# zhenfeizhang/falcon-r1cs

Hardware: AMD Instinct MI355X
Metric: falcon1024_verify_with_ntt_r1cs_witnesses_per_sec (higher is better)
Workload: dtype u32; 1 GPU; falcon-1024 full verify-with-ntt witness (NTT ladder + mod_q + pointwise + l2-norm), batch=65536 signatures per GPU per step (BASELINE configs[2] on every GPU); logn=10, batch_per_gpu=65536, chunk=32768, encoding=bls12-381-fr montgomery (arkworks witness_assignment bytes), seed=0x46414c434f4e31, signatures_failing_range_checks=0, ranks_seen=1, hbm_plan_bytes=166888865792, hbm_plan_limit_bytes=259200000000

## Files before the change

### falcon-r1cs_amd/csrc/frw_layout.h

```cpp
#pragma once
#include <hip/hip_runtime.h>
#include <stddef.h>
#include <stdint.h>

namespace frw {

struct Carve {
    char *base;
    size_t off = 0;
    explicit Carve(void *b) : base((char *)b) {}
    template <class T = void>
    T *take(size_t bytes, size_t align = 256)
    {
        T *p = (T *)(base + off);
        off += (bytes + align - 1) & ~(align - 1);
        return p;
    }
    uint32_t *words(size_t count) { return take<uint32_t>(count * 4, 4); }
    void *at() const { return base + off; }
    void align_to(size_t a) { off = (off + a - 1) & ~(a - 1); }
    static size_t up(size_t bytes, size_t a) { return (bytes + a - 1) & ~(a - 1); }
};

constexpr int MSM_C = 16;
constexpr int MSM_W = 16;
constexpr int MSM_BUCKETS = 1 << (MSM_C - 1);
constexpr int MSM_FOLD1_THREADS = 4096;
constexpr int G1_BK_WORDS = 60, G2_BK_WORDS = 116;
constexpr int MSM_SLICES = 32, MSM_SLICES_LONE = 224;
constexpr int WIDE_C = 20, WIDE_W = 13, WIDE_H = 1 << (WIDE_C - MSM_C), WIDE_ROWS = WIDE_W * WIDE_H;
constexpr uint32_t WIDE_MAX_ITEMS = 65536;
constexpr int WIDE_SLICES = 128;
constexpr int WIDE_BINS = 512, WIDE_BIN_BUCKETS = MSM_BUCKETS * WIDE_H / WIDE_BINS, WIDE_ALL_BINS = WIDE_W * WIDE_BINS, WIDE_TILE = 4096;
constexpr int WIDE_PARTS = 32;
constexpr int MSM_MAX_ITEMS = 131072;
constexpr int MSM_MAX_ITEMS_LARGE = 32768 + (32768 * 24 * 2 / 3) / 32 * 33 + 64;
static_assert(MSM_MAX_ITEMS_LARGE % 64 == 0 && MSM_MAX_ITEMS >= 32768 + (32768 * 4 * 2 / 3) / 32 * 33 + 64, "whole wavefronts; the finest split fits");
__host__ __device__ constexpr uint32_t msm_max_items(uint32_t n, bool bare = false)
{
    return !bare && n > (1u << 18) ? (uint32_t)MSM_MAX_ITEMS_LARGE : (uint32_t)MSM_MAX_ITEMS;
}
constexpr int NMSM_C = 8, NMSM_W = 32, NMSM_BUCKETS = 128;
__host__ __device__ constexpr uint32_t nmsm_slices(uint32_t n) { return n > (1u << 18) ? 128u : 16u; }
constexpr int NMSM_TARGET_ITEMS_MIN = 2048, NMSM_TARGET_ITEMS_MAX = 65536;
__host__ __device__ constexpr uint32_t nmsm_target_items(uint32_t n)
{
    const uint32_t t = (n / 128 + 2047) / 2048 * 2048;
    return t < (uint32_t)NMSM_TARGET_ITEMS_MIN ? (uint32_t)NMSM_TARGET_ITEMS_MIN : t > (uint32_t)NMSM_TARGET_ITEMS_MAX ? (uint32_t)NMSM_TARGET_ITEMS_MAX : t;
}
__host__ __device__ constexpr uint32_t nmsm_max_items(uint32_t n) { return nmsm_target_items(n) + 256; }
constexpr int NMSM_ONES_MAX = 4096, NMSM_ONES_MAX_LARGE = 65536;
__host__ __device__ constexpr uint32_t nmsm_ones_max(uint32_t n) { return n > (1u << 18) ? (uint32_t)NMSM_ONES_MAX_LARGE : (uint32_t)NMSM_ONES_MAX; }

static_assert((size_t)MSM_SLICES * 4 <= (size_t)G1_BK_WORDS * 4, "the slice histograms borrow the buckets' memory");
static_assert((size_t)MSM_SLICES_LONE * MSM_BUCKETS <= (size_t)MSM_MAX_ITEMS * G1_BK_WORDS, "... or, for a lone signature, the work items'");
struct MsmBufs {
    uint32_t *counts, *offsets, *order, *item_first, *item_count, *ones_count, *items, *buckets, *partial, *partial_items, *entries, *ones_list, *end;
    int16_t *digits;
    uint32_t *window_sums;
    uint32_t max_items;
    size_t ent_stride, ones_stride, bytes;
};
inline void msm_layout_head(Carve &c, MsmBufs &b, size_t rows, size_t bw)
{
    b.counts = c.words(rows * MSM_BUCKETS); b.offsets = c.words(rows * MSM_BUCKETS);
    b.order = c.words(rows * MSM_BUCKETS); b.item_first = c.words(rows * MSM_BUCKETS);
    b.item_count = c.words(rows * 4); b.ones_count = c.words(rows * 4);
    b.items = c.words(rows * (size_t)b.max_items * 2);
    b.buckets = c.words(rows * (size_t)MSM_BUCKETS * bw);
    b.partial = c.words(rows * (size_t)MSM_FOLD1_THREADS * bw);
}
inline MsmBufs msm_layout(void *ws, size_t rows, uint32_t n, bool bare, size_t bw)
{
    MsmBufs b{};
    Carve c(ws);
    b.max_items = msm_max_items(n, bare);
    b.ent_stride = bare ? (size_t)n : (size_t)MSM_W * n;
    b.ones_stride = bare ? 0 : (size_t)n;
    msm_layout_head(c, b, rows, bw);
    b.partial_items = c.words(rows * (size_t)b.max_items * bw);
    b.entries = c.words(rows * b.ent_stride);
    b.ones_list = c.words(rows * b.ones_stride);
    if (bare) b.digits = (int16_t *)c.words(((size_t)MSM_W * n * 2 + 3) / 4);
    b.end = (uint32_t *)c.at();
    if (bare) { c.align_to(16); b.window_sums = c.words((size_t)MSM_W * bw); }
    b.bytes = Carve::up(c.off, 16);
    return b;
}
struct MsmWideBufs {
    MsmBufs rows;
    uint32_t *partial_plain, *slice_hist, *bin_count, *row_count, *s1, *s0, *window_sums, *entries, *end;
    unsigned long long *row_start, *bin_start;
    uint2 *coarse;
    int32_t *digits;
    size_t bytes;
};
inline MsmWideBufs msm_layout_wide(void *ws, uint32_t n, size_t bw)
{
    constexpr size_t R = WIDE_ROWS;
    MsmWideBufs w{};
    MsmBufs &b = w.rows;
    Carve c(ws);
    b.max_items = WIDE_MAX_ITEMS;
    msm_layout_head(c, b, R, bw);
    w.partial_plain = c.words(R * (size_t)MSM_FOLD1_THREADS * bw);
    b.partial_items = c.words(R * (size_t)b.max_items * bw);
    w.s1 = c.words(R * bw); w.s0 = c.words(R * bw);
    w.window_sums = c.words((size_t)WIDE_W * bw);
    w.row_start = c.take<unsigned long long>(R * 8, 8);
    w.bin_start = c.take<unsigned long long>((size_t)WIDE_ALL_BINS * 8, 8);
    w.row_count = c.words(R); w.bin_count = c.words(WIDE_ALL_BINS);
    w.slice_hist = c.words((size_t)WIDE_W * WIDE_SLICES * WIDE_BINS);
    w.coarse = (uint2 *)c.words((size_t)WIDE_W * n * 2);
    w.entries = c.words((size_t)WIDE_W * n);
    w.digits = (int32_t *)w.entries;
    w.end = (uint32_t *)c.at();
    b.entries = w.entries; b.ones_list = w.end; b.end = w.end;
    w.bytes = Carve::up(c.off, 16);
    return w;
}
inline size_t msm_workspace_per_signature(uint32_t n, bool bare, bool wide, size_t bw)
{
    return wide ? msm_layout_wide(nullptr, n, bw).bytes : msm_layout(nullptr, bare ? MSM_W : 1, n, bare, bw).bytes;
}

struct NmsmBufs {
    uint32_t *slice_hist, *counts, *offsets, *item_first, *items, *item_count, *ones_count, *ones_list, *entries;
    uint32_t *partial_items, *partial_ones, *folded_ones, *bucket_sums;
    uint32_t target, max_items, ones_stride;
    uint32_t n = 0;
    unsigned long long *entry_base = nullptr;
    uint32_t *window_sums = nullptr;
    uint32_t *end = nullptr;
    size_t used = 0, bytes = 0;
};
inline NmsmBufs nmsm_layout(void *ws, size_t cnt, uint32_t n, size_t bw)
{
    NmsmBufs b;
    Carve c(ws);
    b.target = nmsm_target_items(n); b.max_items = nmsm_max_items(n); b.ones_stride = nmsm_ones_max(n) / 64;
    b.slice_hist = c.words(cnt * (size_t)nmsm_slices(n) * NMSM_BUCKETS);
    b.counts = c.words(cnt * NMSM_BUCKETS);
    b.offsets = c.words(cnt * NMSM_BUCKETS);
    b.item_first = c.words(cnt * NMSM_BUCKETS);
    b.items = c.words(cnt * (size_t)b.max_items);
    b.item_count = c.words(cnt * 4);
    b.ones_count = c.words(cnt * 4);
    b.ones_list = c.words(cnt * (size_t)n);
    b.entries = c.words(cnt * (size_t)NMSM_W * n);
    c.align_to(16);
    b.partial_items = c.words(cnt * (size_t)b.max_items * bw);
    b.partial_ones = c.words(cnt * (size_t)b.ones_stride * bw);
    b.folded_ones = c.words(b.ones_stride > 64 ? cnt * (size_t)64 * bw : 0);
    b.bucket_sums = c.words(cnt * (size_t)NMSM_BUCKETS * bw);
    b.end = (uint32_t *)c.at();
    b.used = c.off;
    b.bytes = Carve::up(c.off + 16, 16);
    return b;
}
inline NmsmBufs nmsm_layout_bare(void *ws, size_t tables, uint32_t n, size_t bw, const NmsmBufs *sorted = nullptr)
{
    constexpr size_t WIN = NMSM_W;
    NmsmBufs b;
    Carve c(ws);
    if (sorted) {
        b = *sorted;
    } else {
        b.target = nmsm_target_items(n); b.max_items = nmsm_max_items(n); b.ones_stride = nmsm_ones_max(n) / 64; b.n = n;
        b.entry_base = c.take<unsigned long long>(WIN * 8, 8);
        b.slice_hist = c.words(WIN * (size_t)nmsm_slices(n) * NMSM_BUCKETS);
        b.counts = c.words(WIN * NMSM_BUCKETS);
        b.offsets = c.words(WIN * NMSM_BUCKETS);
        b.item_first = c.words(WIN * NMSM_BUCKETS);
        b.items = c.words(WIN * (size_t)b.max_items);
        b.item_count = c.words(WIN * 4);
        b.ones_count = c.words(4);
    }
    b.partial_items = c.words(tables * WIN * (size_t)b.max_items * bw);
    b.partial_ones = c.words(tables * (size_t)b.ones_stride * bw);
    b.folded_ones = c.words(tables * (size_t)64 * bw);
    b.bucket_sums = c.words(tables * WIN * (size_t)NMSM_BUCKETS * bw);
    b.window_sums = c.words(tables * WIN * bw);
    if (!sorted) {
        b.ones_list = c.words(n);
        b.entries = c.words(WIN * (size_t)n);
    }
    b.end = (uint32_t *)c.at();
    b.used = c.off;
    b.bytes = Carve::up(c.off + 16, 16);
    return b;
}
inline size_t nmsm_workspace_per_signature(uint32_t n, bool bare, size_t bw) { return bare ? nmsm_layout_bare(nullptr, 1, n, bw).bytes : nmsm_layout(nullptr, 1, n, bw).bytes; }

struct Groth16Points { uint32_t *A, *B1, *L, *H, *SA, *RB1; uint64_t *B2, *rs, *split; };
constexpr size_t GROTH16_POINTS_BYTES = 6 * (size_t)G1_BK_WORDS * 4 + 192 + 64 + 64;
inline Groth16Points groth16_points_layout(Carve &c, size_t cnt)
{
    Groth16Points p;
    p.A = c.words(cnt * G1_BK_WORDS); p.B1 = c.words(cnt * G1_BK_WORDS); p.L = c.words(cnt * G1_BK_WORDS);
    p.H = c.words(cnt * G1_BK_WORDS); p.SA = c.words(cnt * G1_BK_WORDS); p.RB1 = c.words(cnt * G1_BK_WORDS);
    p.B2 = c.take<uint64_t>(cnt * 192, 8); p.rs = c.take<uint64_t>(cnt * 64, 8); p.split = c.take<uint64_t>(cnt * 64, 8);
    return p;
}
struct Groth16Bufs { void *qap_ws; uint64_t *h, *zext; char *msm_ws[5]; Groth16Points pts; size_t qap, msm[5], bytes; };
inline Groth16Bufs groth16_layout(void *ws, size_t cnt, size_t qap, size_t domain, size_t nv, const size_t *msm)
{
    Groth16Bufs g{};
    Carve c(ws);
    g.qap = qap;
    g.qap_ws = c.take(cnt * qap, 1);
    g.h = c.take<uint64_t>(cnt * domain * 32, 1);
    g.zext = c.take<uint64_t>(cnt * (nv + 3) * 32, 1);
    for (int i = 0; i < 5; i++) { g.msm[i] = Carve::up(msm[i], 256); g.msm_ws[i] = c.take<char>(cnt * g.msm[i], 1); }
    g.pts = groth16_points_layout(c, cnt);
    g.bytes = Carve::up(c.off, 256);
    return g;
}
struct Groth16Sides { NmsmBufs g1, gb, g2; };
inline Groth16Sides groth16_sides_layout(Carve &c, uint32_t nz, uint32_t b_rows)
{
    Groth16Sides s;
    s.g1 = nmsm_layout_bare(c.at(), 2, nz, G1_BK_WORDS);              c.take(s.g1.used);
    s.gb = nmsm_layout_bare(c.at(), 1, b_rows, G1_BK_WORDS);          c.take(s.gb.used);
    s.g2 = nmsm_layout_bare(c.at(), 1, b_rows, G2_BK_WORDS, &s.gb);   c.take(s.g2.used);
    return s;
}
struct Groth16BareBufs { void *first_ws; uint64_t *h, *zext; Groth16Sides sides; Groth16Points pts; size_t qap, msm_h, bytes; };
inline Groth16BareBufs groth16_layout_bare(void *ws, size_t qap, size_t msm_h, size_t domain, size_t nv, uint32_t nz, uint32_t b_rows)
{
    Groth16BareBufs g{};
    Carve c(ws);
    g.qap = Carve::up(qap, 256); g.msm_h = Carve::up(msm_h, 256);
    g.first_ws = c.take(g.qap > g.msm_h ? g.qap : g.msm_h, 1);
    g.h = c.take<uint64_t>(domain * 32, 1);
    g.zext = c.take<uint64_t>((nv + 3) * 32, 1);
    g.sides = groth16_sides_layout(c, nz, b_rows);
    g.pts = groth16_points_layout(c, 1);
    g.bytes = Carve::up(c.off, 256);
    return g;
}

struct VerifyBufs { uint64_t *decoded, *prepared; int32_t *decode_status, *status; void *msm_ws, *pairing_ws; size_t msm_bytes, bytes; };
inline VerifyBufs verify_layout(void *ws, size_t k, size_t msm_per, bool bare, size_t proof_bytes = 0, size_t pass_bytes = 0, bool wire = false)
{
    VerifyBufs v{};
    Carve c(ws);
    if (wire) { v.decoded = c.take<uint64_t>(384 * k, 8); v.decode_status = c.take<int32_t>(4 * k, 16); }
    v.msm_bytes = msm_per * (bare ? 1 : k);
    v.msm_ws = c.take(v.msm_bytes, 1);
    v.prepared = c.take<uint64_t>(96 * k, 8);
    v.status = c.take<int32_t>(4 * k, 16);
    v.pairing_ws = c.take(k * proof_bytes + pass_bytes, 1);
    v.bytes = c.off;
    return v;
}
struct RerandBufs { uint64_t *scalars; uint32_t *g1_points, *g2_points; uint64_t *decoded; int32_t *decode_status, *encode_status; size_t bytes; };
constexpr size_t RERAND_SCALAR_BYTES = 128;
inline RerandBufs rerand_layout(void *ws, size_t k, bool wire)
{
    RerandBufs b{};
    Carve c(ws);
    b.scalars = c.take<uint64_t>(k * RERAND_SCALAR_BYTES, 16);
    b.g1_points = c.take<uint32_t>(k * 2 * (size_t)G1_BK_WORDS * 4, 16);
    b.g2_points = c.take<uint32_t>(k * (size_t)G2_BK_WORDS * 4, 16);
    if (wire) {
        b.decoded = c.take<uint64_t>(k * 384, 16);
        b.decode_status = c.take<int32_t>(k * 4, 16);
        b.encode_status = c.take<int32_t>(k * 4, 16);
    }
    b.bytes = c.off;
    return b;
}
struct StatementBufs { uint16_t *pk, *hm; int32_t *decode_status; size_t bytes; };
inline StatementBufs statement_layout(void *ws, int logn, size_t batch)
{
    StatementBufs b{};
    Carve c(ws);
    b.pk = c.take<uint16_t>((batch << logn) * 2, 16);
    b.hm = c.take<uint16_t>((batch << logn) * 2, 16);
    b.decode_status = c.take<int32_t>(batch * 4, 16);
    b.bytes = c.off;
    return b;
}
struct FalconVerifyBufs { uint16_t *sig, *pk, *hm; uint8_t *nonce; int32_t *sig_status, *pk_status; size_t bytes; };
inline FalconVerifyBufs falcon_verify_layout(void *ws, int logn, size_t batch)
{
    FalconVerifyBufs b{};
    Carve c(ws);
    b.sig = c.take<uint16_t>((batch << logn) * 2, 16);
    b.pk = c.take<uint16_t>((batch << logn) * 2, 16);
    b.hm = c.take<uint16_t>((batch << logn) * 2, 16);
    b.nonce = c.take<uint8_t>(batch * 40, 16);
    b.sig_status = c.take<int32_t>(batch * 4, 16);
    b.pk_status = c.take<int32_t>(batch * 4, 16);
    b.bytes = c.off;
    return b;
}
constexpr size_t POK_SCAN_BLOCK = 256;
constexpr size_t POK_WIRE_STAGE = 384;
struct PokProveBufs {
    FalconVerifyBufs screen;
    uint32_t *index, *block_sums, *count;
    uint64_t *rs;
    uint64_t *witness, *instance;
    uint16_t *sig, *pk, *hm;
    uint64_t *proofs;
    uint8_t *wire;
    int32_t *witness_status, *wire_status;
    uint32_t *unsatisfied;
    void *groth16_ws;
    size_t fixed_bytes, per_signature_bytes, groth16_bytes, bytes;
};
inline PokProveBufs pok_prove_layout(void *ws, int logn, size_t batch, size_t k, size_t num_witness, size_t groth16_bytes)
{
    PokProveBufs b{};
    Carve c(ws);
    const size_t n = (size_t)1 << logn;
    b.screen = falcon_verify_layout(c.at(), logn, batch);
    c.take(b.screen.bytes, 16);
    b.index = c.take<uint32_t>(batch * 4, 16);
    b.block_sums = c.take<uint32_t>((batch + POK_SCAN_BLOCK - 1) / POK_SCAN_BLOCK * 4, 16);
    b.count = c.take<uint32_t>(16, 16);
    b.rs = c.take<uint64_t>(batch * 64, 16);
    b.fixed_bytes = c.off;
    c.align_to(256);
    const size_t per0 = c.off;
    b.witness = c.take<uint64_t>(k * num_witness * 32, 256);
    b.instance = c.take<uint64_t>(k * (2 * n + 1) * 32, 16);
    b.sig = c.take<uint16_t>(k * n * 2, 16);
    b.pk = c.take<uint16_t>(k * n * 2, 16);
    b.hm = c.take<uint16_t>(k * n * 2, 16);
    b.proofs = c.take<uint64_t>(k * 384, 16);
    b.wire = c.take<uint8_t>(k * POK_WIRE_STAGE, 16);
    b.witness_status = c.take<int32_t>(k * 4, 16);
    b.wire_status = c.take<int32_t>(k * 4, 16);
    b.unsatisfied = c.take<uint32_t>(k * 4, 16);
    b.per_signature_bytes = c.off - per0;
    c.align_to(256);
    b.groth16_ws = c.take(groth16_bytes, 256);
    b.groth16_bytes = groth16_bytes;
    b.bytes = c.off;
    return b;
}
__host__ __device__ constexpr size_t aggregate_pk_len(int g) { return g ? 1793 : 897; }
__host__ __device__ constexpr size_t aggregate_sig_len(int g) { return g ? 1280 : 666; }
struct AggRoute { size_t pk_off, sig_off, nonce_off; };
__host__ __device__ inline AggRoute aggregate_route(int g, size_t k, size_t s)
{
    const size_t other = s - k;
    AggRoute r;
    r.pk_off = k * aggregate_pk_len(g) + other * aggregate_pk_len(g ^ 1);
    r.sig_off = k * aggregate_sig_len(g) + other * aggregate_sig_len(g ^ 1);
    r.nonce_off = s * 40;
    return r;
}
__host__ __device__ inline size_t aggregate_pk_bytes(size_t count9, size_t count10) { return aggregate_route(0, count9, count9 + count10).pk_off; }
__host__ __device__ inline size_t aggregate_sig_bytes(size_t count9, size_t count10) { return aggregate_route(0, count9, count9 + count10).sig_off; }

struct AggregateScreenBufs {
    uint16_t *sig[2], *pk[2], *hm[2];
    int32_t *sig_status[2], *pk_status[2], *status[2];
    uint64_t *norm[2];
    uint8_t *nonce;
    uint32_t *refused;
    size_t bytes;
};
inline AggregateScreenBufs aggregate_screen_layout(void *ws, size_t count9, size_t count10)
{
    AggregateScreenBufs b{};
    Carve c(ws);
    const size_t count[2] = {count9, count10};
    for (int g = 0; g < 2; g++) {
        const size_t row = count[g] * ((size_t)512 << g) * 2;
        b.sig[g] = c.take<uint16_t>(row, 16);
        b.pk[g] = c.take<uint16_t>(row, 16);
        b.hm[g] = c.take<uint16_t>(row, 16);
        b.sig_status[g] = c.take<int32_t>(count[g] * 4, 16);
        b.pk_status[g] = c.take<int32_t>(count[g] * 4, 16);
        b.status[g] = c.take<int32_t>(count[g] * 4, 16);
        b.norm[g] = c.take<uint64_t>(count[g] * 8, 16);
    }
    b.nonce = c.take<uint8_t>((count9 + count10) * 40, 16);
    b.refused = c.take<uint32_t>(16, 16);
    b.bytes = c.off;
    return b;
}
struct AggregateProveBufs {
    AggregateScreenBufs screen;
    uint64_t *set_witness[2], *set_instance[2];
    int32_t *witness_status[2];
    uint64_t *witness, *instance, *proof;
    uint8_t *wire;
    int32_t *wire_status, *statement_status;
    uint32_t *unsatisfied;
    void *groth16_ws;
    size_t num_witness, num_instance;
    size_t groth16_bytes, bytes;
};
inline AggregateProveBufs aggregate_prove_layout(void *ws, size_t count9, size_t count10, size_t groth16_bytes)
{
    AggregateProveBufs b{};
    Carve c(ws);
    const size_t count[2] = {count9, count10};
    b.screen = aggregate_screen_layout(c.at(), count9, count10);
    c.take(b.screen.bytes, 256);
    b.num_instance = 1;
    for (int g = 0; g < 2; g++) {
        const size_t n = (size_t)512 << g, W = 153 * n + (g ? 52 : 50), I = 2 * n + 1;
        c.align_to(256);
        b.set_witness[g] = c.take<uint64_t>(count[g] * W * 32, 256);
        b.set_instance[g] = c.take<uint64_t>(count[g] * I * 32, 16);
        b.witness_status[g] = c.take<int32_t>(count[g] * 4, 16);
        b.num_witness += count[g] * W;
        b.num_instance += count[g] * (I - 1);
    }
    c.align_to(256);
    b.witness = c.take<uint64_t>(b.num_witness * 32, 256);
    b.instance = c.take<uint64_t>(b.num_instance * 32, 16);
    b.proof = c.take<uint64_t>(384, 16);
    b.wire = c.take<uint8_t>(POK_WIRE_STAGE, 16);
    b.wire_status = c.take<int32_t>(4, 16);
    b.unsatisfied = c.take<uint32_t>(4, 16);
    b.statement_status = c.take<int32_t>((count9 + count10) * 4, 16);
    c.align_to(256);
    b.groth16_ws = c.take(groth16_bytes, 256);
    b.groth16_bytes = groth16_bytes;
    b.bytes = c.off;
    return b;
}
template <class SizeFn> size_t proofs_in_flight(size_t batch, size_t bytes, SizeFn size)
{
    if (batch == 0 || size(1) > bytes) return 0;
    size_t lo = 1, hi = batch;
    while (lo < hi) {
        const size_t mid = lo + (hi - lo + 1) / 2;
        if (size(mid) <= bytes) lo = mid;
        else hi = mid - 1;
    }
    return lo;
}

}
```

### falcon-r1cs_amd/csrc/frw_prepare.hip

```cpp
#include <hip/hip_runtime.h>
#include <stdint.h>
#include <algorithm>
#include "frw_device.h"
#include "frw_keccak.h"
#include "frw_layout.h"

namespace frw {

constexpr int SHAKE256_RATE = 136;
constexpr int NONCE_LEN = 40;

__device__ __forceinline__ void hash_to_point_one(int logn, const uint8_t *__restrict__ nonce, const uint8_t *__restrict__ msg, uint64_t o0,
                                         uint64_t o1, uint16_t *__restrict__ out)
{
    const int n = 1 << logn;
    const size_t total = NONCE_LEN + (size_t)(o1 >= o0 ? o1 - o0 : 0);
    uint64_t st[25];
#pragma unroll
    for (int i = 0; i < 25; i++) st[i] = 0;
    for (size_t pos = 0;; pos += SHAKE256_RATE) {
#pragma unroll
        for (int l = 0; l < SHAKE256_RATE / 8; l++) {
            uint64_t w = 0;
#pragma unroll
            for (int b = 0; b < 8; b++) {
                const size_t p = pos + (size_t)(l * 8 + b);
                uint32_t byte = 0;
                if (p < NONCE_LEN) byte = nonce[p];
                else if (p < total) byte = msg[p - NONCE_LEN];
                else if (p == total) byte = 0x1F;
                w |= (uint64_t)byte << (8 * b);
            }
            st[l] ^= w;
        }
        const bool last = total < pos + SHAKE256_RATE;
        if (last) st[16] ^= 0x8000000000000000ull;
        keccak_f1600(st);
        if (last) break;
    }
    int cnt = 0;
    while (cnt < n) {
#pragma unroll
        for (int w = 0; w < SHAKE256_RATE / 2; w++) {
            const uint64_t lane = st[w / 4];
            const int sh = (w % 4) * 16;
            const uint32_t v = (uint32_t)((lane >> sh) & 0xff) << 8 | (uint32_t)((lane >> (sh + 8)) & 0xff);
            if (v < 5 * Q && cnt < n) out[cnt++] = (uint16_t)(v % Q);
        }
        if (cnt < n) keccak_f1600(st);
    }
}

__global__ __launch_bounds__(BLOCK) void hash_to_point_kernel(int logn, size_t batch, const uint8_t *__restrict__ nonces,
                                                              const uint8_t *__restrict__ msgs,
                                                              const uint64_t *__restrict__ msg_off, uint16_t *__restrict__ hm)
{
    const size_t s = (size_t)blockIdx.x * blockDim.x + threadIdx.x;
    if (s >= batch) return;
    const uint64_t o0 = msg_off[s], o1 = msg_off[s + 1];
    hash_to_point_one(logn, nonces + s * NONCE_LEN, msgs + o0, o0, o1, hm + (s << logn));
}

__device__ __forceinline__ uint32_t public_key_coeff(const uint8_t *__restrict__ p, int k)
{
    const int bit = 14 * k, off = bit & 7;
    const uint8_t *q = p + 1 + (bit >> 3);
    uint32_t acc = (uint32_t)q[0] << 16 | (uint32_t)q[1] << 8;
    if (off + 14 > 16) acc |= q[2];
    return (acc >> (24 - 14 - off)) & 0x3fffu;
}

__global__ __launch_bounds__(BLOCK) void decode_public_keys_kernel(int logn, size_t batch, const uint8_t *__restrict__ pk_bytes,
                                                                   uint16_t *__restrict__ pk, int32_t *__restrict__ status)
{
    const int n = 1 << logn;
    const size_t pk_len = 1 + (size_t)14 * n / 8;
    const size_t idx = (size_t)blockIdx.x * blockDim.x + threadIdx.x;
    if (idx >= batch * (size_t)n) return;
    const size_t s = idx >> logn;
    const int k = (int)(idx & (size_t)(n - 1));
    const uint8_t *p = pk_bytes + s * pk_len;
    const uint32_t c = public_key_coeff(p, k);
    pk[idx] = (uint16_t)c;
    if (c >= Q || (k == 0 && p[0] != (uint8_t)logn)) atomicMax(&status[s], ST_DECODE);
}

__device__ __forceinline__ bool decode_signature_one(int logn, const uint8_t *__restrict__ p, size_t sig_len, uint16_t *__restrict__ out,
                                            uint8_t *__restrict__ nonce_out)
{
    const int n = 1 << logn;
    bool ok = sig_len > 1 + NONCE_LEN && p[0] == (uint8_t)(0x30 + logn);
    if (ok && nonce_out)
        for (int i = 0; i < NONCE_LEN; i++) nonce_out[i] = p[1 + i];
    const uint8_t *body = p + 1 + NONCE_LEN;
    const size_t body_len = ok ? sig_len - 1 - NONCE_LEN : 0;
    size_t v = 0;
    uint32_t acc = 0;
    int acc_len = 0;
    for (int u = 0; ok && u < n; u++) {
        if (v >= body_len) { ok = false; break; }
        acc = (acc << 8) | body[v++];
        const uint32_t b = acc >> acc_len;
        const uint32_t sign = b & 128u;
        uint32_t m = b & 127u;
        for (;;) {
            if (acc_len == 0) {
                if (v >= body_len) { ok = false; break; }
                acc = (acc << 8) | body[v++];
                acc_len = 8;
            }
            acc_len--;
            if ((acc >> acc_len) & 1u) break;
            m += 128;
            if (m > 2047) { ok = false; break; }
        }
        if (sign && m == 0) ok = false;
        if (ok) out[u] = (uint16_t)(sign ? Q - m : m);
    }
    if (ok && (acc & ((1u << acc_len) - 1u))) ok = false;
    for (; ok && v < body_len; v++)
        if (body[v]) ok = false;
    return ok;
}

__global__ __launch_bounds__(BLOCK) void decode_signatures_kernel(int logn, size_t batch, const uint8_t *__restrict__ sig_bytes,
                                                                  size_t sig_len, uint16_t *__restrict__ sig,
                                                                  uint8_t *__restrict__ nonce_out, int32_t *__restrict__ status)
{
    const size_t s = (size_t)blockIdx.x * blockDim.x + threadIdx.x;
    if (s >= batch) return;
    const bool ok = decode_signature_one(logn, sig_bytes + s * sig_len, sig_len, sig + (s << logn),
                                         nonce_out ? nonce_out + s * NONCE_LEN : nullptr);
    status[s] = ok ? ST_OK : ST_DECODE;
}

__global__ __launch_bounds__(BLOCK) void agg_hash_to_point_kernel(int logn, size_t count, const uint32_t *__restrict__ stmt,
                                                                  const uint8_t *__restrict__ nonces, const uint8_t *__restrict__ msgs,
                                                                  const uint64_t *__restrict__ msg_off, uint16_t *__restrict__ hm)
{
    const size_t k = (size_t)blockIdx.x * blockDim.x + threadIdx.x;
    if (k >= count) return;
    const size_t s = stmt[k];
    const uint64_t o0 = msg_off[s], o1 = msg_off[s + 1];
    hash_to_point_one(logn, nonces + aggregate_route(logn - 9, k, s).nonce_off, msgs + o0, o0, o1, hm + (k << logn));
}

__global__ __launch_bounds__(BLOCK) void agg_decode_public_keys_kernel(int logn, size_t count, const uint32_t *__restrict__ stmt,
                                                                       const uint8_t *__restrict__ pk_bytes, uint16_t *__restrict__ pk,
                                                                       int32_t *__restrict__ status)
{
    const int n = 1 << logn;
    const size_t idx = (size_t)blockIdx.x * blockDim.x + threadIdx.x;
    if (idx >= count * (size_t)n) return;
    const size_t k = idx >> logn;
    const int j = (int)(idx & (size_t)(n - 1));
    const uint8_t *p = pk_bytes + aggregate_route(logn - 9, k, stmt[k]).pk_off;
    const uint32_t c = public_key_coeff(p, j);
    pk[idx] = (uint16_t)c;
    if (c >= Q || (j == 0 && p[0] != (uint8_t)logn)) atomicMax(&status[k], ST_DECODE);
}

__global__ __launch_bounds__(BLOCK) void agg_decode_signatures_kernel(int logn, size_t count, const uint32_t *__restrict__ stmt,
                                                                      const uint8_t *__restrict__ sig_bytes, uint16_t *__restrict__ sig,
                                                                      uint8_t *__restrict__ nonces, int32_t *__restrict__ status)
{
    const size_t k = (size_t)blockIdx.x * blockDim.x + threadIdx.x;
    if (k >= count) return;
    const AggRoute r = aggregate_route(logn - 9, k, stmt[k]);
    const uint8_t *p = sig_bytes + r.sig_off;
    for (int i = 0; i < NONCE_LEN; i++) nonces[r.nonce_off + i] = p[1 + i];
    status[k] = decode_signature_one(logn, p, aggregate_sig_len(logn - 9), sig + (k << logn), nullptr) ? ST_OK : ST_DECODE;
}

struct AggVerdicts { const uint32_t *stmt[2]; const int32_t *status[2]; const uint64_t *norm[2]; uint32_t count[2]; };
__global__ __launch_bounds__(BLOCK) void agg_scatter_verdicts_kernel(AggVerdicts v, int32_t *__restrict__ status, uint64_t *__restrict__ norm)
{
    size_t k = (size_t)blockIdx.x * blockDim.x + threadIdx.x;
    int g = 0;
    if (k >= v.count[0]) { k -= v.count[0]; g = 1; }
    if (k >= v.count[g]) return;
    const size_t s = v.stmt[g][k];
    status[s] = v.status[g][k];
    if (norm) norm[s] = v.norm[g][k];
}

__global__ __launch_bounds__(BLOCK) void agg_count_refused_kernel(size_t count, const int32_t *__restrict__ status, uint32_t *__restrict__ refused)
{
    __shared__ uint32_t wave_count[WAVES];
    uint32_t mine = 0;
    for (size_t s = threadIdx.x; s < count; s += BLOCK) mine += status[s] != ST_OK;
#pragma unroll
    for (int off = WAVE / 2; off > 0; off >>= 1) mine += __shfl_xor(mine, off, WAVE);
    if ((threadIdx.x & (WAVE - 1)) == 0) wave_count[threadIdx.x / WAVE] = mine;
    __syncthreads();
    if (threadIdx.x == 0) {
        uint32_t total = 0;
#pragma unroll
        for (int w = 0; w < WAVES; w++) total += wave_count[w];
        refused[0] = total;
    }
}


__device__ inline uint32_t pok_block_rank(bool flag, uint32_t &total)
{
    __shared__ uint32_t wave_count[WAVES];
    const uint64_t mask = __ballot(flag);
    const int lane = threadIdx.x & (WAVE - 1), wave = threadIdx.x / WAVE;
    if (lane == 0) wave_count[wave] = (uint32_t)__popcll(mask);
    __syncthreads();
    uint32_t before = 0;
    total = 0;
#pragma unroll
    for (int w = 0; w < WAVES; w++) {
        if (w < wave) before += wave_count[w];
        total += wave_count[w];
    }
    return before + (uint32_t)__popcll(mask & (((uint64_t)1 << lane) - 1));
}

__global__ __launch_bounds__(BLOCK) void pok_scan_count_kernel(size_t batch, const int32_t *__restrict__ status,
                                                               uint32_t *__restrict__ block_sums)
{
    const size_t s = (size_t)blockIdx.x * BLOCK + threadIdx.x;
    uint32_t total;
    (void)pok_block_rank(s < batch && status[s] == ST_OK, total);
    if (threadIdx.x == 0) block_sums[blockIdx.x] = total;
}

__global__ __launch_bounds__(BLOCK) void pok_scan_offsets_kernel(size_t num_blocks, uint32_t *__restrict__ block_sums,
                                                                 uint32_t *__restrict__ count)
{
    __shared__ uint32_t wave_sum[WAVES];
    const int lane = threadIdx.x & (WAVE - 1), wave = threadIdx.x / WAVE;
    uint32_t carry = 0;
    for (size_t base = 0; base < num_blocks; base += BLOCK) {
        const size_t i = base + threadIdx.x;
        const uint32_t v = i < num_blocks ? block_sums[i] : 0;
        uint32_t incl = v;
#pragma unroll
        for (int d = 1; d < WAVE; d <<= 1) {
            const uint32_t up = __shfl_up(incl, d, WAVE);
            if (lane >= d) incl += up;
        }
        if (lane == WAVE - 1) wave_sum[wave] = incl;
        __syncthreads();
        uint32_t before = 0, tile = 0;
#pragma unroll
        for (int w = 0; w < WAVES; w++) {
            if (w < wave) before += wave_sum[w];
            tile += wave_sum[w];
        }
        if (i < num_blocks) block_sums[i] = carry + before + incl - v;
        carry += tile;
        __syncthreads();
    }
    if (threadIdx.x == 0) count[0] = carry;
}

__global__ __launch_bounds__(BLOCK) void pok_scan_write_kernel(size_t batch, const int32_t *__restrict__ status,
                                                               const uint32_t *__restrict__ block_offsets, uint32_t *__restrict__ index)
{
    const size_t s = (size_t)blockIdx.x * BLOCK + threadIdx.x;
    const bool ok = s < batch && status[s] == ST_OK;
    uint32_t total;
    const uint32_t rank = pok_block_rank(ok, total);
    if (ok) index[block_offsets[blockIdx.x] + rank] = (uint32_t)s;
}

__global__ __launch_bounds__(BLOCK) void pok_gather_rs_kernel(size_t count, const uint32_t *__restrict__ index,
                                                              const uint64_t *__restrict__ rs, uint64_t *__restrict__ dense_rs)
{
    const size_t t = (size_t)blockIdx.x * BLOCK + threadIdx.x;
    if (t >= count * 8) return;
    dense_rs[t] = rs[(size_t)index[t / 8] * 8 + (t & 7)];
}

__global__ __launch_bounds__(BLOCK) void pok_gather_inputs_kernel(int logn, const uint32_t *__restrict__ index,
                                                                  const uint16_t *__restrict__ sig, const uint16_t *__restrict__ pk,
                                                                  const uint16_t *__restrict__ hm, uint16_t *__restrict__ sig_out,
                                                                  uint16_t *__restrict__ pk_out, uint16_t *__restrict__ hm_out)
{
    const size_t j = blockIdx.x, slot = index[j];
    const uint32_t row = (2u << logn) / 16;
    for (uint32_t t = threadIdx.x; t < 3 * row; t += BLOCK) {
        const uint32_t a = t / row, v = t % row;
        const uint16_t *src = a == 0 ? sig : a == 1 ? pk : hm;
        uint16_t *dst = a == 0 ? sig_out : a == 1 ? pk_out : hm_out;
        ((uint4 *)dst)[j * row + v] = ((const uint4 *)src)[slot * row + v];
    }
}

struct PokOutputs { uint8_t *wire; uint64_t *proofs, *instance; uint32_t *unsatisfied; uint32_t wire_len, inst_words; };

__global__ __launch_bounds__(BLOCK) void pok_zero_refused_kernel(size_t batch, const int32_t *__restrict__ status, PokOutputs out)
{
    for (size_t s = blockIdx.x; s < batch; s += gridDim.x) {
        if (status[s] == ST_OK) continue;
        for (uint32_t t = threadIdx.x; t < out.wire_len; t += BLOCK) out.wire[s * out.wire_len + t] = 0;
        if (out.proofs && threadIdx.x < 48) out.proofs[s * 48 + threadIdx.x] = 0;
        if (out.instance)
            for (uint32_t t = threadIdx.x; t < out.inst_words; t += BLOCK) out.instance[s * out.inst_words + t] = 0;
        if (out.unsatisfied && threadIdx.x == 0) out.unsatisfied[s] = 0;
    }
}

__global__ __launch_bounds__(BLOCK) void pok_scatter_kernel(const uint32_t *__restrict__ index, const uint8_t *__restrict__ wire,
                                                            const uint64_t *__restrict__ proofs, const uint64_t *__restrict__ instance,
                                                            const uint32_t *__restrict__ unsatisfied, PokOutputs out)
{
    const size_t j = blockIdx.x, s = index[j];
    for (uint32_t t = threadIdx.x; t < out.wire_len; t += BLOCK) out.wire[s * out.wire_len + t] = wire[j * out.wire_len + t];
    if (out.proofs && threadIdx.x < 48) out.proofs[s * 48 + threadIdx.x] = proofs[j * 48 + threadIdx.x];
    if (out.instance)
        for (uint32_t t = threadIdx.x; t < out.inst_words; t += BLOCK) out.instance[s * out.inst_words + t] = instance[j * out.inst_words + t];
    if (out.unsatisfied && threadIdx.x == 0) out.unsatisfied[s] = unsatisfied[j];
}

hipError_t launch_pok_scan(size_t batch, const int32_t *status, uint32_t *block_sums, uint32_t *index, uint32_t *count, hipStream_t st)
{
    if (batch == 0) return hipSuccess;
    const size_t blocks = (batch + BLOCK - 1) / BLOCK;
    hipLaunchKernelGGL(pok_scan_count_kernel, dim3((unsigned)blocks), dim3(BLOCK), 0, st, batch, status, block_sums);
    hipLaunchKernelGGL(pok_scan_offsets_kernel, dim3(1), dim3(BLOCK), 0, st, blocks, block_sums, count);
    hipLaunchKernelGGL(pok_scan_write_kernel, dim3((unsigned)blocks), dim3(BLOCK), 0, st, batch, status, (const uint32_t *)block_sums, index);
    return hipGetLastError();
}

hipError_t launch_pok_gather_rs(size_t count, const uint32_t *index, const uint64_t *rs, uint64_t *dense_rs, hipStream_t st)
{
    if (count == 0) return hipSuccess;
    hipLaunchKernelGGL(pok_gather_rs_kernel, dim3((unsigned)((count * 8 + BLOCK - 1) / BLOCK)), dim3(BLOCK), 0, st, count, index, rs, dense_rs);
    return hipGetLastError();
}

hipError_t launch_pok_gather_inputs(int logn, size_t cnt, const uint32_t *index, const uint16_t *sig, const uint16_t *pk, const uint16_t *hm,
                                    uint16_t *sig_out, uint16_t *pk_out, uint16_t *hm_out, hipStream_t st)
{
    if (cnt == 0) return hipSuccess;
    hipLaunchKernelGGL(pok_gather_inputs_kernel, dim3((unsigned)cnt), dim3(BLOCK), 0, st, logn, index, sig, pk, hm, sig_out, pk_out, hm_out);
    return hipGetLastError();
}

hipError_t launch_pok_zero_refused(size_t batch, const int32_t *status, int wire_len, int inst_words, uint8_t *wire, uint64_t *proofs,
                                   uint64_t *instance, uint32_t *unsatisfied, hipStream_t st)
{
    if (batch == 0) return hipSuccess;
    const PokOutputs out = {wire, proofs, instance, unsatisfied, (uint32_t)wire_len, (uint32_t)inst_words};
    hipLaunchKernelGGL(pok_zero_refused_kernel, dim3((unsigned)std::min<size_t>(batch, 65536)), dim3(BLOCK), 0, st, batch, status, out);
    return hipGetLastError();
}

hipError_t launch_pok_scatter(size_t cnt, const uint32_t *index, int wire_len, int inst_words, const uint8_t *wire_in,
                              const uint64_t *proofs_in, const uint64_t *instance_in, const uint32_t *unsatisfied_in, uint8_t *wire,
                              uint64_t *proofs, uint64_t *instance, uint32_t *unsatisfied, hipStream_t st)
{
    if (cnt == 0) return hipSuccess;
    const PokOutputs out = {wire, proofs, instance, unsatisfied, (uint32_t)wire_len, (uint32_t)inst_words};
    hipLaunchKernelGGL(pok_scatter_kernel, dim3((unsigned)cnt), dim3(BLOCK), 0, st, index, wire_in, proofs_in, instance_in, unsatisfied_in, out);
    return hipGetLastError();
}

hipError_t launch_hash_to_point(int logn, size_t batch, const uint8_t *nonces, const uint8_t *msgs, const uint64_t *msg_off,
                                uint16_t *hm, hipStream_t st)
{
    if (batch == 0) return hipSuccess;
    hipLaunchKernelGGL(hash_to_point_kernel, dim3((unsigned)((batch + BLOCK - 1) / BLOCK)), dim3(BLOCK), 0, st, logn, batch, nonces,
                       msgs, msg_off, hm);
    return hipGetLastError();
}

hipError_t launch_decode_public_keys(int logn, size_t batch, const uint8_t *pk_bytes, uint16_t *pk, int32_t *status, hipStream_t st)
{
    if (batch == 0) return hipSuccess;
    hipError_t e = hipMemsetAsync(status, 0, batch * sizeof(int32_t), st);
    if (e != hipSuccess) return e;
    const size_t total = batch << logn;
    hipLaunchKernelGGL(decode_public_keys_kernel, dim3((unsigned)((total + BLOCK - 1) / BLOCK)), dim3(BLOCK), 0, st, logn, batch,
                       pk_bytes, pk, status);
    return hipGetLastError();
}

hipError_t launch_decode_signatures(int logn, size_t batch, const uint8_t *sig_bytes, size_t sig_len, uint16_t *sig,
                                    uint8_t *nonce_out, int32_t *status, hipStream_t st)
{
    if (batch == 0) return hipSuccess;
    hipLaunchKernelGGL(decode_signatures_kernel, dim3((unsigned)((batch + BLOCK - 1) / BLOCK)), dim3(BLOCK), 0, st, logn, batch,
                       sig_bytes, sig_len, sig, nonce_out, status);
    return hipGetLastError();
}

hipError_t launch_agg_hash_to_point(int logn, size_t count, const uint32_t *stmt, const uint8_t *nonces, const uint8_t *msgs,
                                    const uint64_t *msg_off, uint16_t *hm, hipStream_t st)
{
    if (count == 0) return hipSuccess;
    hipLaunchKernelGGL(agg_hash_to_point_kernel, dim3((unsigned)((count + BLOCK - 1) / BLOCK)), dim3(BLOCK), 0, st, logn, count, stmt, nonces,
                       msgs, msg_off, hm);
    return hipGetLastError();
}

hipError_t launch_agg_decode_public_keys(int logn, size_t count, const uint32_t *stmt, const uint8_t *pk_bytes, uint16_t *pk, int32_t *status,
                                         hipStream_t st)
{
    if (count == 0) return hipSuccess;
    hipError_t e = hipMemsetAsync(status, 0, count * sizeof(int32_t), st);
    if (e != hipSuccess) return e;
    const size_t total = count << logn;
    hipLaunchKernelGGL(agg_decode_public_keys_kernel, dim3((unsigned)((total + BLOCK - 1) / BLOCK)), dim3(BLOCK), 0, st, logn, count, stmt,
                       pk_bytes, pk, status);
    return hipGetLastError();
}

hipError_t launch_agg_decode_signatures(int logn, size_t count, const uint32_t *stmt, const uint8_t *sig_bytes, uint16_t *sig, uint8_t *nonces,
                                        int32_t *status, hipStream_t st)
{
    if (count == 0) return hipSuccess;
    hipLaunchKernelGGL(agg_decode_signatures_kernel, dim3((unsigned)((count + BLOCK - 1) / BLOCK)), dim3(BLOCK), 0, st, logn, count, stmt,
                       sig_bytes, sig, nonces, status);
    return hipGetLastError();
}

hipError_t launch_agg_verdicts(const uint32_t *const stmt[2], const int32_t *const set_status[2], const uint64_t *const set_norm[2],
                               const size_t count[2], int32_t *status, uint64_t *norm, uint32_t *refused, hipStream_t st)
{
    const size_t total = count[0] + count[1];
    if (total == 0) return hipSuccess;
    const AggVerdicts v = {{stmt[0], stmt[1]}, {set_status[0], set_status[1]}, {set_norm[0], set_norm[1]}, {(uint32_t)count[0], (uint32_t)count[1]}};
    hipLaunchKernelGGL(agg_scatter_verdicts_kernel, dim3((unsigned)((total + BLOCK - 1) / BLOCK)), dim3(BLOCK), 0, st, v, status, norm);
    hipLaunchKernelGGL(agg_count_refused_kernel, dim3(1), dim3(BLOCK), 0, st, total, (const int32_t *)status, refused);
    return hipGetLastError();
}

}
```

Baseline: 1.348 million signatures/s.

## Stage hash-to-point and signature decode through LDS with coalesced I/O

Rewrites hash_to_point and decode_signatures as one-wave-per-block kernels. Input bytes are staged cooperatively into LDS with 16-byte loads, and outputs are written through LDS tiles and rings as coalesced uint4 stores, replacing the per-thread strided global accesses. Signature decoding also switches to a 64-bit bit accumulator that uses clz to read the unary part. The cost is extra barriers, a large LDS footprint that limits occupancy, and more complex edge handling for misaligned buffers.

Result: no change. 1.347 million signatures/s (-0.1%).

```diff
diff --git a/falcon-r1cs_amd/csrc/frw_layout.h b/falcon-r1cs_amd/csrc/frw_layout.h
--- a/falcon-r1cs_amd/csrc/frw_layout.h
+++ b/falcon-r1cs_amd/csrc/frw_layout.h
@@ -428,6 +428,34 @@
     b.bytes = c.off;
     return b;
 }
+constexpr uint32_t SIG_STAGE_LDS_BYTES = 53248;
+constexpr uint32_t SIG_STAGE_MAX_ROWS = 64;
+constexpr uint32_t SIG_TILE_COEFFS = 64, SIG_TILE_PITCH_DW = SIG_TILE_COEFFS / 2 + 1;
+struct SigStagePlan { uint32_t chunks, pitch_dw, rows; };
+__host__ __device__ inline SigStagePlan sig_stage_plan(size_t sig_len)
+{
+    SigStagePlan p{0, 0, 0};
+    if (sig_len > SIG_STAGE_LDS_BYTES) return p;
+    p.chunks = (uint32_t)((sig_len + 15 + 15) / 16);
+    p.pitch_dw = 4 * p.chunks + 1;
+    const uint32_t per_row = (p.pitch_dw + SIG_TILE_PITCH_DW) * 4;
+    p.rows = SIG_STAGE_LDS_BYTES / per_row;
+    if (p.rows > SIG_STAGE_MAX_ROWS) p.rows = SIG_STAGE_MAX_ROWS;
+    return p;
+}
+struct SigStageChunk { size_t src; uint32_t dst, len; };
+__host__ __device__ inline SigStageChunk sig_stage_chunk(uint32_t align, size_t batch, size_t sig_len, size_t s, uint32_t k)
+{
+    const size_t a = align + s * sig_len, end = align + batch * sig_len;
+    const size_t c0 = (a & ~(size_t)15) + (size_t)16 * k;
+    SigStageChunk c{0, 16 * k, 0};
+    if (c0 >= a + sig_len) return c;
+    if (c0 >= align && c0 + 16 <= end) { c.src = c0 - align; c.len = 16; return c; }
+    const size_t lo = c0 > a ? c0 : a, hi = c0 + 16 < a + sig_len ? c0 + 16 : a + sig_len;
+    c.src = lo - align; c.dst += (uint32_t)(lo - c0); c.len = (uint32_t)(hi - lo);
+    return c;
+}
+
 template <class SizeFn> size_t proofs_in_flight(size_t batch, size_t bytes, SizeFn size)
 {
     if (batch == 0 || size(1) > bytes) return 0;
diff --git a/falcon-r1cs_amd/csrc/frw_prepare.hip b/falcon-r1cs_amd/csrc/frw_prepare.hip
--- a/falcon-r1cs_amd/csrc/frw_prepare.hip
+++ b/falcon-r1cs_amd/csrc/frw_prepare.hip
@@ -51,14 +51,96 @@
     }
 }
 
-__global__ __launch_bounds__(BLOCK) void hash_to_point_kernel(int logn, size_t batch, const uint8_t *__restrict__ nonces,
-                                                              const uint8_t *__restrict__ msgs,
-                                                              const uint64_t *__restrict__ msg_off, uint16_t *__restrict__ hm)
-{
-    const size_t s = (size_t)blockIdx.x * blockDim.x + threadIdx.x;
-    if (s >= batch) return;
-    const uint64_t o0 = msg_off[s], o1 = msg_off[s + 1];
-    hash_to_point_one(logn, nonces + s * NONCE_LEN, msgs + o0, o0, o1, hm + (s << logn));
+constexpr uint32_t HASH_RING = 256, HASH_RING_PITCH_DW = HASH_RING / 2 + 1, HASH_BLOCK_PITCH_DW = SHAKE256_RATE / 4 + 1;
+__global__ __launch_bounds__(WAVE) void hash_to_point_kernel(int logn, size_t batch, const uint8_t *__restrict__ nonces,
+                                                             const uint8_t *__restrict__ msgs,
+                                                             const uint64_t *__restrict__ msg_off, uint16_t *__restrict__ hm)
+{
+    __shared__ uint32_t lds[WAVE * HASH_RING_PITCH_DW];
+    __shared__ uint64_t row_o0[WAVE], row_total[WAVE];
+    const uint32_t lane = threadIdx.x;
+    const uint32_t n = 1u << logn;
+    const size_t s0 = (size_t)blockIdx.x * WAVE;
+    const uint32_t rows = (uint32_t)(batch - s0 < WAVE ? batch - s0 : WAVE);
+    const bool mine = lane < rows;
+    uint64_t total = 0;
+    if (mine) {
+        const uint64_t o0 = msg_off[s0 + lane], o1 = msg_off[s0 + lane + 1];
+        total = NONCE_LEN + (o1 >= o0 ? o1 - o0 : 0);
+        row_o0[lane] = o0;
+        row_total[lane] = total;
+    }
+    uint64_t st[25];
+#pragma unroll
+    for (int i = 0; i < 25; i++) st[i] = 0;
+    __syncthreads();
+
+    uint8_t *const block_bytes = (uint8_t *)lds;
+    const uint64_t last_block = total / SHAKE256_RATE;
+    for (uint64_t blk = 0;; blk++) {
+        const bool absorbing = mine && blk <= last_block;
+        const uint64_t rows_in = __ballot(absorbing);
+        if (!rows_in) break;
+        const uint64_t pos0 = blk * SHAKE256_RATE;
+        for (uint32_t i = lane; i < rows * SHAKE256_RATE; i += WAVE) {
+            const uint32_t r = i / SHAKE256_RATE, p = i - r * SHAKE256_RATE;
+            if (!((rows_in >> r) & 1)) continue;
+            const uint64_t pos = pos0 + p, tot = row_total[r];
+            uint32_t byte = 0;
+            if (pos < NONCE_LEN) byte = nonces[(s0 + r) * NONCE_LEN + pos];
+            else if (pos < tot) byte = msgs[row_o0[r] + (pos - NONCE_LEN)];
+            else if (pos == tot) byte = 0x1F;
+            if (p == SHAKE256_RATE - 1 && tot < pos0 + SHAKE256_RATE) byte ^= 0x80;
+            block_bytes[r * (HASH_BLOCK_PITCH_DW * 4) + p] = (uint8_t)byte;
+        }
+        __syncthreads();
+        if (absorbing) {
+            const uint32_t *b = lds + lane * HASH_BLOCK_PITCH_DW;
+#pragma unroll
+            for (int l = 0; l < SHAKE256_RATE / 8; l++) st[l] ^= (uint64_t)b[2 * l] | (uint64_t)b[2 * l + 1] << 32;
+            keccak_f1600(st);
+        }
+        __syncthreads();
+    }
+
+    uint16_t *const ring = (uint16_t *)lds + lane * (HASH_RING_PITCH_DW * 2);
+    const bool wide_out = ((uintptr_t)hm & 15) == 0;
+    uint32_t cnt = mine ? 0 : n, flushed = 0;
+    for (;;) {
+        const bool go = cnt < n && cnt - flushed + SHAKE256_RATE / 2 <= HASH_RING;
+        if (go) {
+#pragma unroll
+            for (int w = 0; w < SHAKE256_RATE / 2; w++) {
+                const uint64_t word = st[w / 4];
+                const int sh = (w % 4) * 16;
+                const uint32_t v = (uint32_t)((word >> sh) & 0xff) << 8 | (uint32_t)((word >> (sh + 8)) & 0xff);
+                if (v < 5 * Q && cnt < n) { ring[cnt & (HASH_RING - 1)] = (uint16_t)(v % Q); cnt++; }
+            }
+        }
+        uint32_t low = cnt;
+#pragma unroll
+        for (int off = WAVE / 2; off > 0; off >>= 1) low = min(low, (uint32_t)__shfl_xor((int)low, off, WAVE));
+        const uint32_t upto = low & ~31u;
+        __syncthreads();
+        if (upto > flushed) {
+            if (wide_out) {
+                const uint32_t per_row = (upto - flushed) / 8;
+                for (uint32_t i = lane; i < rows * per_row; i += WAVE) {
+                    const uint32_t r = i / per_row, c = flushed + 8 * (i - r * per_row);
+                    const uint32_t *src = lds + r * HASH_RING_PITCH_DW + (c & (HASH_RING - 1)) / 2;
+                    *(uint4 *)(hm + ((s0 + r) << logn) + c) = make_uint4(src[0], src[1], src[2], src[3]);
+                }
+            } else {
+                for (uint32_t r = 0; r < rows; r++)
+                    for (uint32_t c = flushed + lane; c < upto; c += WAVE)
+                        hm[((s0 + r) << logn) + c] = ((const uint16_t *)lds)[r * (HASH_RING_PITCH_DW * 2) + (c & (HASH_RING - 1))];
+            }
+            flushed = upto;
+        }
+        __syncthreads();
+        if (low >= n) break;
+        if (go && cnt < n) keccak_f1600(st);
+    }
 }
 
 __device__ __forceinline__ uint32_t public_key_coeff(const uint8_t *__restrict__ p, int k)
@@ -123,15 +205,131 @@
     return ok;
 }
 
-__global__ __launch_bounds__(BLOCK) void decode_signatures_kernel(int logn, size_t batch, const uint8_t *__restrict__ sig_bytes,
-                                                                  size_t sig_len, uint16_t *__restrict__ sig,
-                                                                  uint8_t *__restrict__ nonce_out, int32_t *__restrict__ status)
-{
-    const size_t s = (size_t)blockIdx.x * blockDim.x + threadIdx.x;
-    if (s >= batch) return;
-    const bool ok = decode_signature_one(logn, sig_bytes + s * sig_len, sig_len, sig + (s << logn),
-                                         nonce_out ? nonce_out + s * NONCE_LEN : nullptr);
-    status[s] = ok ? ST_OK : ST_DECODE;
+__global__ __launch_bounds__(WAVE) void decode_signatures_kernel(int logn, size_t batch, const uint8_t *__restrict__ sig_bytes,
+                                                                 size_t sig_len, uint16_t *__restrict__ sig,
+                                                                 uint8_t *__restrict__ nonce_out, int32_t *__restrict__ status)
+{
+    __shared__ uint32_t lds[SIG_STAGE_LDS_BYTES / 4];
+    const uint32_t lane = threadIdx.x;
+    const SigStagePlan plan = sig_stage_plan(sig_len);
+    if (plan.rows == 0 || sig_len <= 1 + NONCE_LEN) {
+        const size_t s = (size_t)blockIdx.x * WAVE + lane;
+        if (s >= batch) return;
+        const bool ok = decode_signature_one(logn, sig_bytes + s * sig_len, sig_len, sig + (s << logn),
+                                             nonce_out ? nonce_out + s * NONCE_LEN : nullptr);
+        status[s] = ok ? ST_OK : ST_DECODE;
+        return;
+    }
+    const int n = 1 << logn;
+    const size_t s0 = (size_t)blockIdx.x * plan.rows;
+    const uint32_t rows = (uint32_t)(batch - s0 < plan.rows ? batch - s0 : plan.rows);
+    const uint32_t align = (uint32_t)((uintptr_t)sig_bytes & 15);
+    uint8_t *const lds_bytes = (uint8_t *)lds;
+    uint16_t *const tile = (uint16_t *)(lds + plan.rows * plan.pitch_dw);
+
+    constexpr int IN_FLIGHT = 4;
+    const uint32_t items = rows * plan.chunks;
+    for (uint32_t i0 = lane; i0 < items; i0 += IN_FLIGHT * WAVE) {
+        SigStageChunk c[IN_FLIGHT];
+        uint4 v[IN_FLIGHT];
+        uint32_t at[IN_FLIGHT];
+#pragma unroll
+        for (int q = 0; q < IN_FLIGHT; q++) {
+            const uint32_t i = i0 + q * WAVE;
+            c[q].len = 0;
+            if (i < items) {
+                const uint32_t r = i / plan.chunks, k = i - r * plan.chunks;
+                c[q] = sig_stage_chunk(align, batch, sig_len, s0 + r, k);
+                at[q] = r * plan.pitch_dw + 4 * k;
+                if (c[q].len == 16) v[q] = *(const uint4 *)(sig_bytes + c[q].src);
+            }
+        }
+#pragma unroll
+        for (int q = 0; q < IN_FLIGHT; q++) {
+            if (c[q].len == 16) {
+                uint32_t *d = lds + at[q];
+                d[0] = v[q].x; d[1] = v[q].y; d[2] = v[q].z; d[3] = v[q].w;
+            } else {
+                for (uint32_t b = 0; b < c[q].len; b++) lds_bytes[(size_t)at[q] * 4 + (c[q].dst & 15) + b] = sig_bytes[c[q].src + b];
+            }
+        }
+    }
+    __syncthreads();
+
+    const uint32_t phase = (uint32_t)((align + (s0 + lane) * sig_len) & 15);
+    const uint32_t b0 = phase + 1 + NONCE_LEN, body_len = (uint32_t)sig_len - 1 - NONCE_LEN;
+    const uint32_t d0 = b0 >> 2, body_dwords = ((b0 & 3) + body_len + 3) >> 2;
+    const uint32_t *const body = lds + lane * plan.pitch_dw + d0;
+    auto masked_dword = [&](uint32_t j) -> uint32_t {
+        if (j >= body_dwords) return 0;
+        uint32_t w = __builtin_bswap32(body[j]);
+        if (j == 0) w &= 0xffffffffu >> (8 * (b0 & 3));
+        const uint32_t left = (b0 & 3) + body_len - 4 * j;
+        if (left < 4) w &= 0xffffffffu << (8 * (4 - left));
+        return w;
+    };
+    const bool mine = lane < rows;
+    const bool header = mine && lds_bytes[(size_t)lane * plan.pitch_dw * 4 + phase] == (uint8_t)(0x30 + logn);
+    bool ok = header;
+    const uint32_t total_bits = 8 * body_len;
+    uint64_t acc = 0;
+    uint32_t acc_len = 0, pos = 0;
+    uint32_t next = 0, ahead = 0;
+    if (ok) { acc = masked_dword(0); acc_len = 32 - 8 * (b0 & 3); ahead = __builtin_bswap32(body[1]); next = 2; }
+    const bool wide_out = ((uintptr_t)sig & 15) == 0;
+    for (int t = 0; t < n; t += (int)SIG_TILE_COEFFS) {
+        if (ok) {
+            uint16_t *const mine_out = tile + lane * (SIG_TILE_PITCH_DW * 2);
+            for (uint32_t u = 0; u < SIG_TILE_COEFFS; u++) {
+                if (acc_len < 32) {
+                    acc = (acc << 32) | ahead;
+                    acc_len += 32;
+                    ahead = __builtin_bswap32(body[next < body_dwords ? next : body_dwords]);
+                    next++;
+                }
+                const uint32_t x = (uint32_t)(acc >> (acc_len - 32));
+                const uint32_t zeros = (uint32_t)__builtin_clz((x << 8) | 0x8000u);
+                const uint32_t m = ((x >> 24) & 127u) + (zeros << 7);
+                const uint32_t used = 9 + zeros;
+                pos += used;
+                if (zeros > 15 || pos > total_bits || ((x >> 31) && m == 0)) { ok = false; break; }
+                acc_len -= used;
+                mine_out[u] = (uint16_t)((x >> 31) ? Q - m : m);
+            }
+        }
+        const uint64_t alive = __ballot(ok);
+        __syncthreads();
+        if (wide_out) {
+            for (uint32_t p = 0; p < rows; p += 8) {
+                const uint32_t r = p + (lane >> 3), seg = lane & 7;
+                if (r < rows && ((alive >> r) & 1)) {
+                    const uint32_t *src = (const uint32_t *)tile + r * SIG_TILE_PITCH_DW + 4 * seg;
+                    *(uint4 *)(sig + ((s0 + r) << logn) + t + 8 * seg) = make_uint4(src[0], src[1], src[2], src[3]);
+                }
+            }
+        } else {
+            for (uint32_t r = 0; r < rows; r++)
+                if ((alive >> r) & 1) sig[((s0 + r) << logn) + t + lane] = tile[r * (SIG_TILE_PITCH_DW * 2) + lane];
+        }
+        __syncthreads();
+        if (!alive) break;
+    }
+    if (ok) {
+        const uint32_t left = total_bits - pos, held = left < acc_len ? left : acc_len;
+        if ((acc >> (acc_len - held)) & (((uint64_t)1 << held) - 1)) ok = false;
+        for (uint32_t j = next - 1; ok && j < body_dwords; j++)
+            if (masked_dword(j)) ok = false;
+    }
+    if (mine) status[s0 + lane] = ok ? ST_OK : ST_DECODE;
+
+    if (nonce_out) {
+        const uint64_t expected = __ballot(header);
+        for (uint32_t i = lane; i < rows * NONCE_LEN; i += WAVE) {
+            const uint32_t r = i / NONCE_LEN, b = i - r * NONCE_LEN;
+            const uint32_t ph = (uint32_t)((align + (s0 + r) * sig_len) & 15);
+            if ((expected >> r) & 1) nonce_out[s0 * NONCE_LEN + i] = lds_bytes[(size_t)r * plan.pitch_dw * 4 + ph + 1 + b];
+        }
+    }
 }
 
 __global__ __launch_bounds__(BLOCK) void agg_hash_to_point_kernel(int logn, size_t count, const uint32_t *__restrict__ stmt,
@@ -365,7 +563,7 @@
                                 uint16_t *hm, hipStream_t st)
 {
     if (batch == 0) return hipSuccess;
-    hipLaunchKernelGGL(hash_to_point_kernel, dim3((unsigned)((batch + BLOCK - 1) / BLOCK)), dim3(BLOCK), 0, st, logn, batch, nonces,
+    hipLaunchKernelGGL(hash_to_point_kernel, dim3((unsigned)((batch + WAVE - 1) / WAVE)), dim3(WAVE), 0, st, logn, batch, nonces,
                        msgs, msg_off, hm);
     return hipGetLastError();
 }
@@ -385,7 +583,9 @@
                                     uint8_t *nonce_out, int32_t *status, hipStream_t st)
 {
     if (batch == 0) return hipSuccess;
-    hipLaunchKernelGGL(decode_signatures_kernel, dim3((unsigned)((batch + BLOCK - 1) / BLOCK)), dim3(BLOCK), 0, st, logn, batch,
+    const SigStagePlan plan = sig_stage_plan(sig_len);
+    const size_t per = plan.rows == 0 || sig_len <= 1 + NONCE_LEN ? (size_t)WAVE : plan.rows;
+    hipLaunchKernelGGL(decode_signatures_kernel, dim3((unsigned)((batch + per - 1) / per)), dim3(WAVE), 0, st, logn, batch,
                        sig_bytes, sig_len, sig, nonce_out, status);
     return hipGetLastError();
 }
```
